# thanosDelatolas/eva-vos

Hardware: AMD Instinct MI355X
Metric: frames/sec STCN mask-propagate 480p 1-obj (higher is better)
Workload: dtype f32; 1 GPU; DAVIS-17-val-shaped 480x854 (padded 480x864) single-object STCN propagate: fresh engine, interact(mask,0), T=66 frames/video, mem_freq=5, top_k=50; one video per step per GPU; videos_per_gpu=38, streams_per_gpu=4, key_lookahead=0, clips=8 distinct synthetic clips (one per pooled engine), weights=synthetic recipe seed 0 (no checkpoints offline)

## Files before the change

eva_vos_amd/csrc/engine.cpp:

```cpp
#include "engine.h"
#include "src_hash.h"

#include <algorithm>
#include <atomic>
#include <cmath>
#include <cstdarg>
#include <cstdio>
#include <cstdlib>
#include <cstring>
#include <map>
#include <mutex>
#include <unordered_map>
#include <utility>

namespace stcn {

static thread_local char g_err[512] = "";
void set_error(const char *fmt, ...) {
    va_list ap;
    va_start(ap, fmt);
    vsnprintf(g_err, sizeof(g_err), fmt, ap);
    va_end(ap);
}
const char *get_error() { return g_err; }

Knobs Knobs::from_env() {
    Knobs k;
    k.wino_min_cin = env_int("STCN_WINO_MIN_CIN", k.wino_min_cin);
    k.wino_ppw = env_int("STCN_WINO_PPW", k.wino_ppw);
    k.wino4_chunk_mb = env_int("STCN_WINO4_CHUNK_MB", k.wino4_chunk_mb);
    k.fusion_conv12 = env_int("STCN_FUSION_CONV12", k.fusion_conv12) != 0;
    k.fusion_wino = env_int("STCN_FUSION_WINO", k.fusion_wino) != 0;
    k.pw_chain = env_int("STCN_PW_CHAIN", k.pw_chain);
    return k;
}

void Prof::reset() {
    for (int i = 0; i < STCN_K_COUNT; ++i) { flops[i] = 0; bytes[i] = 0; exec_flops[i] = 0; launches[i] = 0; }
    hbm_conv_flops = hbm_conv_bytes = hbm_conv_ms = 0; hbm_conv_launches = 0;
    wino2_flops = wino4_flops = 0;
    for (auto &e : events) { pool.push_back(e.a); pool.push_back(e.b); }
    events.clear();
}
Prof::Ev &Prof::push_pair(int cls, bool hbm) {
    Ev e; e.cls = cls; e.hbm = hbm;
    for (hipEvent_t *p : {&e.a, &e.b}) {
        if (!pool.empty()) { *p = pool.back(); pool.pop_back(); }
        else (void)hipEventCreate(p);
// ... 357 lines not shown
    if ((rc = alloc((void **)&logit4, (size_t)kg * d.hw4 * sizeof(float)))) return rc;
    if ((rc = alloc((void **)&flogit, (size_t)k * d.npix * sizeof(float)))) return rc;
    if ((rc = alloc((void **)&agg, (size_t)(k + 1) * group * d.npix * sizeof(float)))) return rc;
    if ((rc = alloc((void **)&agg_alt, (size_t)(k + 1) * group * d.npix * sizeof(float)))) return rc;
    if ((rc = alloc((void **)&pooled, (size_t)std::max(20, attention_nchp(2 * (k + 1))) * d.hw16 * sizeof(float)))) return rc;
    if ((rc = alloc((void **)&amap, (size_t)(k + 1) * 2 * d.hw16 * sizeof(float)))) return rc;
    if ((rc = alloc((void **)&attn, (size_t)(k + 1) * 2 * d.npix * sizeof(float)))) return rc;
    const MemReadScratchSizes ms = memread_scratch_floats(group * d.hw16);
    if ((rc = alloc((void **)&cand_v, std::max(ms.cand_v, attention_part_floats(k + 1, d.hw16)) * sizeof(float)))) return rc;
    if ((rc = alloc((void **)&cand_i, ms.cand_i * sizeof(int32_t)))) return rc;
    if ((rc = alloc((void **)&cand_n, ms.cand_n * sizeof(int32_t)))) return rc;
    if ((rc = alloc((void **)&qk, (size_t)group * d.hw16 * 64 * sizeof(float)))) return rc;
    if ((rc = alloc((void **)&vin, (size_t)k * d.npix * 8 * sizeof(float)))) return rc;
    if ((rc = alloc((void **)&gmax, ms.gmax * sizeof(float)))) return rc;
    if ((rc = alloc((void **)&tau, ms.tau * sizeof(float)))) return rc;
    return STCN_OK;
}
void Work::release() {
    for (void *p : allocs) pool_free(p);
    allocs.clear();
}

static thread_local int g_fail_countdown = 0;
static thread_local int g_fail_reserve = 0;
static std::atomic<int> g_side_delay_us{0};
void inject_failure_after(int n) { g_fail_countdown = n; }
int launch_status(const char *what) {
    if (g_fail_countdown > 0 && --g_fail_countdown == 0) {
        (void)hipGetLastError();
        set_error("launch of '%s' failed: injected fault (stcn_test_fail_at)", what);
// ... 54 lines not shown
    p.x0_bytes = (unsigned)x0b;
    p.x1_bytes = (unsigned)x1b;
    p.w_bytes = (unsigned)((long)cw.cout * cw.Kp * 4);
    if (a.x1 && ((cw.cin_p % 32) || (c0 % 32) || cw.kh * cw.kw > 32)) { set_error("conv '%s': two-source input needs 32-aligned channel splits", name.c_str()); return STCN_E_INVALID; }
    p.w = cw.w; p.wino_u = cw.wino_u; p.wino4_u = cw.wino4_u;
    p.bias = cw.bias; p.res = a.res; p.res_bs = res_bs; p.res_bmod = a.res_bmod; p.y = a.y; p.y_bs = a.y_bs;
    p.relu_in = a.relu_in; p.relu_out = a.relu_out;
    p.fd_ohw = fastdiv_make((unsigned)(p.OH * p.OW));
    p.fd_ow = fastdiv_make((unsigned)p.OW);
    p.fd_cin = fastdiv_make((unsigned)p.Cin);
    p.fd_kw = fastdiv_make((unsigned)p.KW);
    p.pointwise = cw.kh == 1 && cw.kw == 1 && a.stride == 1 && !a.x1 && bs0 == (long)H * W * c0;
    p.affine_out = (a.y_bs == 0 || a.y_bs == (long)p.OH * p.OW * p.N) && (!a.res || (res_bs == (long)p.OH * p.OW * p.N && !a.res_bmod)) &&
                   ((long)p.M + 128) * p.N * 4 < (1L << 32);
    p.partial = w.splitk;
    p.kn = w.kn;
    pl = ConvPlan{};
    pl.fl = 2.0 * p.M * p.N * (double)(cw.kh * cw.kw * cw.cin);
    if (a.force_splitk <= 0 && (fusion_conv_plan(p, pl) || wino4_plan(p, m.wino4_min_wg, w.wino_v_floats, w.splitk_floats, pl) ||
                                wino_plan(p, w.wino_v_floats, w.splitk_floats, pl)))
        return STCN_OK;
    conv_plan(p, a.force_splitk, w.splitk_floats, pl);
    return STCN_OK;
}

int run_conv(const Model &m, Work &w, hipStream_t s, const std::string &name, const ConvArgs &a) {
    ConvP p;
    ConvPlan &pl = g_path.plan;
    const int rc = plan_conv(m, w, name, a, p, pl);
    if (rc) return rc;
// ... 485 lines not shown
    if (rc) { stcn_engine_destroy(e); return rc; }
    const Dims &d = e->d;
    for (int t = 0; t < T; ++t)
        pack_image_launch(images_dev + (size_t)t * 3 * H * W, e->images4 + (size_t)t * d.npix * 4, H, W, nh, nw, e->lw, e->lh, e->stream);
    if ((rc = engine_init_outputs(e))) { stcn_engine_destroy(e); return rc; }
    HIPCHK(hipStreamSynchronize(e->stream));
    *out = e;
    return STCN_OK;
}

int stcn_engine_reset(stcn_engine *e) {
    if (!e) { set_error("stcn_engine_reset: null engine"); return STCN_E_INVALID; }
    HIPCHK(hipSetDevice(e->model->device));
    if (e->side) HIPCHK(hipStreamSynchronize(e->side));
    if (e->stream2) HIPCHK(hipStreamSynchronize(e->stream2));
    e->failed.clear();
    e->interacted.clear();
    e->n_certain = 0;
    e->n_cached = 0;
    std::fill(e->slot_of.begin(), e->slot_of.end(), -1);
    std::fill(e->vparts_ready.begin(), e->vparts_ready.end(), 0);
    std::fill(e->key_pending.begin(), e->key_pending.end(), 0);
    e->fuse_pending[0] = e->fuse_pending[1] = 0;
    e->stats = stcn_stats{};
    return engine_init_outputs(e);
}

int stcn_engine_destroy(stcn_engine *e) {
    if (!e) return STCN_OK;
    if (e->stream) (void)hipStreamSynchronize(e->stream); else (void)hipDeviceSynchronize();
// ... 458 lines not shown
```

eva_vos_amd/csrc/engine.h:

```cpp
#pragma once
#include <hip/hip_runtime.h>

#include <deque>
#include <map>
#include <memory>
#include <set>
#include <string>
#include <vector>

#include "../../include/stcn_hip.h"
#include "kernels.h"

namespace stcn {

void set_error(const char *fmt, ...);
struct Model;
struct ConvW;
hipError_t pool_malloc(void **p, size_t bytes);
void pool_free(void *p);
void pool_release();
bool wants_wino(const ConvW &cw);
bool wants_wino4(const ConvW &cw);
bool wants_wino_fusion12(const ConvW &cw);
int make_wino(Model &m, ConvW &cw, const std::vector<float> &w_host);
// ... 69 lines not shown
    float *A = nullptr, *B = nullptr, *C = nullptr, *D = nullptr;
    float *splitk = nullptr; size_t splitk_floats = 0;
    float *wino_v = nullptr; size_t wino_v_floats = 0;
    float *cbam = nullptr;
    float *readout = nullptr;
    float *logit4 = nullptr;
    float *flogit = nullptr;
    float *agg = nullptr;
    float *agg_alt = nullptr;
    float *pooled = nullptr, *amap = nullptr, *attn = nullptr;
    float *cand_v = nullptr; int32_t *cand_i = nullptr, *cand_n = nullptr;
    float *gmax = nullptr, *tau = nullptr;
    int32_t *centre = nullptr;
    float *qk = nullptr;
    float *vin = nullptr;
    Prof *prof = nullptr;
    Knobs kn = Knobs::from_env();
    int conv_cls = STCN_K_CONV;
    std::vector<void *> allocs;
    int init(int nh, int nw, int k, int key_batch = 1, int group = 1);
    void release();
};

struct KeyOut { float *k16, *msq, *f16_thin, *f16, *s8, *s4, *f8_copy, *f4_copy, *dthin = nullptr, *cthin = nullptr; };
void inject_failure_after(int n);
int launch_status(const char *what);
const char *last_conv_path();
void set_conv_path(const char *s);
void conv_trace(int on);
const char *conv_trace_get();
constexpr long CONV_DENSE = -1;
struct ConvArgs {
    const float *x0 = nullptr, *x1 = nullptr;
    int c0 = 0, c1 = 0;
    long bs0 = CONV_DENSE, bs1 = 0;
    int B = 1, H = 0, W = 0, stride = 1;
// ... 86 lines not shown
```

eva_vos_amd/csrc/hooks.cpp:

```cpp
#include <algorithm>
#include <cmath>
#include <cstdlib>
#include <cstring>
#include <string>
#include <vector>

#include "engine.h"

using namespace stcn;
#define RC(x) do { int rc_ = (x); if (rc_) return rc_; } while (0)

namespace {
struct TmpWork {
    Work w;
    int rc;
    TmpWork(int nh, int nw, int k) { rc = w.init(nh, nw, k); }
    ~TmpWork() { (void)hipDeviceSynchronize(); w.release(); }
};
struct DevBuf {
    float *p = nullptr;
    int alloc(size_t floats) { HIPCHK(hipMalloc((void **)&p, floats * 4)); return STCN_OK; }
    ~DevBuf() { if (p) { (void)hipDeviceSynchronize(); (void)hipFree(p); } }
};
ConvW test_convw(int Cin, int Cout, int KH, int KW) {
    ConvW cw;
    cw.cout = Cout; cw.cin = Cin; cw.cin_p = Cin; cw.kh = KH; cw.kw = KW;
    cw.K = KH * KW * Cin; cw.Kp = (cw.K + 31) / 32 * 32;
    return cw;
}
size_t test_wino_v_floats(int B, int OH, int OW, int Cin) {
    const size_t v2 = (size_t)16 * Cin * (((size_t)B * ((OH + 1) / 2) * ((OW + 1) / 2) + 63) / 64 * 64);
    const size_t v4 = (size_t)36 * Cin * (((size_t)B * ((OH + 3) / 4) * ((OW + 3) / 4) + 127) / 128 * 128);
    return v2 > v4 ? v2 : v4;
}
struct ConvRig {
    Model m;
    Work w;
    DevBuf wv, ws;
    ~ConvRig() { (void)hipDeviceSynchronize(); for (void *p : m.allocs) (void)hipFree(p); }
    int init(ConvW cw, const std::vector<float> *hw, bool f4, int B, int OH, int OW, size_t slab_floats) {
        if (hw) {
            RC(make_wino(m, cw, *hw));
            RC(make_wino_fusion12(m, cw, *hw));
            if (f4) RC(make_wino4(m, cw, *hw));
            w.wino_v_floats = test_wino_v_floats(B, OH, OW, cw.cin_p);
            RC(wv.alloc(w.wino_v_floats));
            w.wino_v = wv.p;
        }
        m.conv["t"] = cw;
        w.splitk_floats = slab_floats;
        RC(ws.alloc(w.splitk_floats));
        w.splitk = ws.p;
        return STCN_OK;
    }
};
int plan_test_conv(int B, int H, int W, int Cin, int Cout, int K, int stride, int flags, int splitk, ConvP &p, ConvPlan &pl) {
    static float buf[4];
    Model m;
    ConvW cw = test_convw(Cin, Cout, K, K);
    cw.w = cw.bias = buf;
    const int OH = (H + 2 * (K / 2) - K) / stride + 1, OW = (W + 2 * (K / 2) - K) / stride + 1;
    Work w;
    if (K == 3 && stride == 1) {
        if (wants_wino(cw) || wants_wino_fusion12(cw)) cw.wino_u = buf;
        if (flags & 4) { if (wants_wino4(cw)) cw.wino4_u = buf; m.wino4_min_wg = 0; }
        w.wino_v_floats = test_wino_v_floats(B, OH, OW, Cin);
        w.wino_v = buf;
// ... 370 lines not shown
```

eva_vos_amd/csrc/kernels.h:

```cpp
#pragma once
#include <hip/hip_runtime.h>
#include <stdint.h>

#include <cstdlib>

#include "../../include/stcn_hip.h"

namespace stcn {

struct FastDiv {
    unsigned magic, shift, d;
};
static inline FastDiv fastdiv_make(unsigned d) {
    FastDiv f{0, 0, d};
    if (d <= 1) return f;
    unsigned s = 0;
    while ((1ull << s) < d) ++s;
    f.magic = (unsigned)(((1ull << (31 + s)) / d) + 1);
    f.shift = s - 1;
    return f;
}
#if defined(__HIPCC__)
__device__ __forceinline__ int fastdiv(int x, const FastDiv f) {
    return f.d <= 1 ? x : (int)(__umulhi((unsigned)x, f.magic) >> f.shift);
// ... 3 lines not shown
    return (xcd < r8 ? xcd * (q8 + 1) : r8 * (q8 + 1) + (xcd - r8) * q8) + (bid >> 3);
}
#endif

static inline int env_int(const char *name, int dflt) { const char *e = getenv(name); return e ? atoi(e) : dflt; }
static inline bool env_on(const char *name, bool dflt = true) { return env_int(name, dflt) != 0; }
int device_cus();

struct Knobs {
    int wino_min_cin = 128;
    int wino_ppw = 0;
    int wino4_chunk_mb = 160;
    int fusion_conv12 = 0;
    int fusion_wino = 1;
    int pw_chain = 2;
    static Knobs from_env();
};

struct ConvP {
    const float *x0, *x1;
    int c0, c1;
    long bs0, bs1;
    unsigned x0_bytes, x1_bytes, w_bytes;
    int B, H, W;
    int OH, OW;
    int KH, KW, stride, pad;
    int Cin;
    int M, N;
    int K, Kp;
    const float *w;
    const float *bias;
    const float *res;
    long res_bs;
    int res_bmod;
    float *y;
    long y_bs;
    int relu_in, relu_out;
    int splitk;
    float *partial;
    int rem_full, rem_split, rem_per;
    const float *wino_u;
    const float *wino4_u;
    FastDiv fd_ohw, fd_ow;
    FastDiv fd_cin, fd_kw;
    int pointwise;
    int affine_out;
    int tile_big;
    int panel;
    int chain;
    Knobs kn;
};
constexpr int W4_MAX_CHUNKS = 16;
struct WinoGeom { int TH, TW, Mt, Mt_pad, KB; };
struct W2Plan { int tiles_n, ntile, kb_per_split; };
struct W4Plan { int tiles_m, tiles_n, mb, grid, full_wg, pieces, per, chunks, tm_per_chunk, judge_wg; };
enum ConvFamily { CONV_LITERAL = 0, CONV_FUSION = 1, CONV_WINO4 = 2, CONV_WINO2 = 3, CONV_DIRECT = 4 };
struct ConvPlan {
    int family = CONV_LITERAL;
    bool fusion_wino = false;
    WinoGeom geo{};
    W4Plan w4{};
    W2Plan w2{};
    int splitk = 1;
    int ppw = 0;
    const char *variant = "";
    bool tail = false;
// ... 109 lines not shown
```

eva_vos_amd/csrc/winograd4.hip:

```cpp
#include <hip/hip_ext.h>

#include <cstdio>
#include <cstdlib>
#include <type_traits>

#include "wino_common.h"

namespace stcn {

typedef float f32x4 __attribute__((ext_vector_type(4)));
typedef float f32x16 __attribute__((ext_vector_type(16)));

#ifdef STCN_W4_CLOCK
__device__ unsigned long long g_w4_clock[2 * 8192];
#if STCN_W4_CLOCK == 2
#define W4_MFMA(a_, b_, c_) w4_fake_mfma(a_, b_, c_)
#endif
#endif
#ifndef W4_MFMA
#define W4_MFMA(a_, b_, c_) __builtin_amdgcn_mfma_f32_32x32x2f32(a_, b_, c_, 0, 0, 0)
#endif

static constexpr int W4T = 32;
static constexpr int W4N = 32;
// ... 72 lines not shown
}

struct Wino4G {
    const float *V, *U;
    unsigned v_bytes, u_bytes;
    int Mt, Mt_pad, KB, N;
    int TH, TW, OH, OW, B, M;
    const float *bias, *res;
    long res_bs; int res_bmod;
    float *y; long y_bs;
    int relu_out;
    FastDiv fd_tpi, fd_tw, fd_tiles_n;
    int full_wg, pieces, kb_per_piece;
    float *partial;
    int tm0;
    int xb_m, xb_n, xb_cols;
};

template <int MB>
__global__ __launch_bounds__(64 * W4W) void wino4_gemm_kernel(const Wino4G p, const int tiles_n) {
    constexpr int PPW = 3, WT = W4T * MB;
    extern __shared__ __attribute__((aligned(16))) float smem[];
    int swz, piece = -1, kb0 = 0, kb1 = p.KB;
    if (MB == 1 && p.pieces > 1 && (int)blockIdx.x >= p.full_wg) {
        const int j = xcd_contiguous_block((int)blockIdx.x - p.full_wg, (int)gridDim.x - p.full_wg);
        const int rt = j / p.pieces;
        piece = j - rt * p.pieces;
        swz = p.full_wg + rt;
        kb0 = piece * p.kb_per_piece;
        kb1 = min(p.KB, kb0 + p.kb_per_piece);
    } else {
        swz = xcd_contiguous_block((int)blockIdx.x, MB == 1 && p.pieces > 1 ? p.full_wg : (int)gridDim.x);
    }
    int tm_l = fastdiv(swz, p.fd_tiles_n), tn = swz - tm_l * tiles_n;
    if (p.xb_m > 0 && piece < 0) {
        const int per = p.xb_m * p.xb_n, blk = swz / per, in = swz - blk * per;
        const int bm_i = blk / p.xb_cols, bn_i = blk - bm_i * p.xb_cols, im = in / p.xb_n;
        tm_l = bm_i * p.xb_m + im;
        tn = bn_i * p.xb_n + (in - im * p.xb_n);
    }
    const int tm = tm_l + p.tm0;
    const int t = threadIdx.x, lane = t & 63, l31 = lane & 31, h = lane >> 5;
    const int wave = __builtin_amdgcn_readfirstlane(t >> 6);
    const int pos0 = PPW * wave;

    const __amdgpu_buffer_rsrc_t rv = __builtin_amdgcn_make_buffer_rsrc(const_cast<float *>(p.V), 0, p.v_bytes, 0x00020000);
    const __amdgpu_buffer_rsrc_t ru = __builtin_amdgcn_make_buffer_rsrc(const_cast<float *>(p.U), 0, p.u_bytes, 0x00020000);
    const unsigned vl = (unsigned)(l31 * 32 + h * 16);
    unsigned sa0[PPW], sb0[PPW];
#pragma unroll
    for (int pi = 0; pi < PPW; ++pi) {
        sa0[pi] = (unsigned)((((long)(pos0 + pi) * p.KB + kb0) * p.Mt_pad + tm * WT) * 32);
        sb0[pi] = (unsigned)((((long)(pos0 + pi) * p.KB + kb0) * p.N + tn * W4N) * 32);
    }
    const unsigned sa = (unsigned)p.Mt_pad * 32u, sb = (unsigned)p.N * 32u;

    f32x16 acc[PPW][MB];
#pragma unroll
    for (int pi = 0; pi < PPW; ++pi)
#pragma unroll
        for (int bi = 0; bi < MB; ++bi)
#pragma unroll
            for (int e = 0; e < 16; ++e) acc[pi][bi][e] = 0.f;

    const int nk = kb1 - kb0;
    auto load1 = [&](int k, int pi, f32x4 (&fa)[MB], f32x4 &fb) {
        const unsigned oa = sa0[pi] + (unsigned)k * sa, ob = sb0[pi] + (unsigned)k * sb;
#pragma unroll
        for (int bi = 0; bi < MB; ++bi) fa[bi] = __builtin_bit_cast(f32x4, __builtin_amdgcn_raw_buffer_load_b128(rv, vl, oa + bi * 1024u, 0));
        fb = __builtin_bit_cast(f32x4, __builtin_amdgcn_raw_buffer_load_b128(ru, vl, ob, 0));
    };
    auto compute1 = [&](int pi, const f32x4 (&fa)[MB], const f32x4 &fb) {
#pragma unroll
        for (int j = 0; j < 4; ++j)
#pragma unroll
            for (int bi = 0; bi < MB; ++bi) acc[pi][bi] = W4_MFMA(fa[bi][j], fb[j], acc[pi][bi]);
    };
#ifdef STCN_W4_CLOCK
    unsigned long long ck_t0 = 0, ck_r0 = 0;
    if (wave == 0) {
        __builtin_amdgcn_sched_barrier(0);
        ck_t0 = __builtin_amdgcn_s_memtime();
        ck_r0 = __builtin_amdgcn_s_memrealtime();
        __builtin_amdgcn_s_waitcnt(0xC07F);
        __builtin_amdgcn_sched_barrier(0);
    }
#endif
    if (MB == 1) {
        f32x4 fa[3][PPW][MB], fb[3][PPW];
        auto load = [&](int k, int set) {
#pragma unroll
            for (int pi = 0; pi < PPW; ++pi) load1(k, pi, fa[set][pi], fb[set][pi]);
        };
        auto compute = [&](int set) {
#pragma unroll
            for (int j = 0; j < 4; ++j)
#pragma unroll
                for (int pi = 0; pi < PPW; ++pi)
#pragma unroll
                    for (int bi = 0; bi < MB; ++bi)
                        acc[pi][bi] = W4_MFMA(fa[set][pi][bi][j], fb[set][pi][j], acc[pi][bi]);
        };
        load(0, 0);
        load(min(1, nk - 1), 1);
        int k = 0;
        for (; k + 2 < nk; k += 3) {
            load(k + 2, 2);
            __builtin_amdgcn_sched_barrier(0);
            compute(0);
            __builtin_amdgcn_sched_barrier(0);
            load(min(k + 3, nk - 1), 0);
            __builtin_amdgcn_sched_barrier(0);
            compute(1);
            __builtin_amdgcn_sched_barrier(0);
            load(min(k + 4, nk - 1), 1);
            __builtin_amdgcn_sched_barrier(0);
            compute(2);
            __builtin_amdgcn_sched_barrier(0);
        }
        if (k < nk) compute(0);
        if (k + 1 < nk) compute(1);
    } else {
        f32x4 fa[2][PPW], fb[2][PPW];
        auto loadA = [&](int k, int bi, f32x4 (&d)[PPW]) {
#pragma unroll
            for (int pi = 0; pi < PPW; ++pi)
                d[pi] = __builtin_bit_cast(f32x4, __builtin_amdgcn_raw_buffer_load_b128(rv, vl, sa0[pi] + (unsigned)k * sa + bi * 1024u, 0));
        };
        auto loadB = [&](int k, f32x4 (&d)[PPW]) {
#pragma unroll
            for (int pi = 0; pi < PPW; ++pi)
                d[pi] = __builtin_bit_cast(f32x4, __builtin_amdgcn_raw_buffer_load_b128(ru, vl, sb0[pi] + (unsigned)k * sb, 0));
        };
        auto comp = [&](int bi, const f32x4 (&a)[PPW], const f32x4 (&bb)[PPW]) {
#pragma unroll
            for (int j = 0; j < 4; ++j)
#pragma unroll
                for (int pi = 0; pi < PPW; ++pi) acc[pi][bi] = W4_MFMA(a[pi][j], bb[pi][j], acc[pi][bi]);
        };
        loadB(0, fb[0]);
        loadA(0, 0, fa[0]);
        for (int k = 0; k < nk; k += 2) {
            const int k2 = min(k + 2, nk - 2);
            loadA(k, 1, fa[1]);
            __builtin_amdgcn_sched_barrier(0);
            comp(0, fa[0], fb[0]);
            __builtin_amdgcn_sched_barrier(0);
            loadB(k + 1, fb[1]);
            loadA(k + 1, 0, fa[0]);
            __builtin_amdgcn_sched_barrier(0);
            comp(1, fa[1], fb[0]);
            __builtin_amdgcn_sched_barrier(0);
            loadA(k + 1, 1, fa[1]);
            __builtin_amdgcn_sched_barrier(0);
            comp(0, fa[0], fb[1]);
            __builtin_amdgcn_sched_barrier(0);
            loadB(k2, fb[0]);
            loadA(k2, 0, fa[0]);
            __builtin_amdgcn_sched_barrier(0);
            comp(1, fa[1], fb[1]);
            __builtin_amdgcn_sched_barrier(0);
        }
    }
#ifdef STCN_W4_CLOCK
    if (wave == 0) {
        __builtin_amdgcn_sched_barrier(0);
        const unsigned long long ck_t1 = __builtin_amdgcn_s_memtime(), ck_r1 = __builtin_amdgcn_s_memrealtime();
        __builtin_amdgcn_s_waitcnt(0xC07F);
        __builtin_amdgcn_sched_barrier(0);
        if (lane == 0 && blockIdx.x < 8192) { g_w4_clock[2 * blockIdx.x] = ck_t1 - ck_t0; g_w4_clock[2 * blockIdx.x + 1] = ck_r1 - ck_r0; }
    }
#endif
    const int chq = t & 7, tl = (t >> 3) & 31;
    const int jh = __builtin_amdgcn_readfirstlane(t >> 8);
    const int tpi = p.TH * p.TW, ohw = p.OH * p.OW;
    const int n = tn * W4N + 4 * chq;
    const bool kpiece = MB == 1 && piece >= 0;
    const float lo = p.relu_out ? 0.f : -__builtin_inff();
    const __amdgpu_buffer_rsrc_t rres = __builtin_amdgcn_make_buffer_rsrc(const_cast<float *>(p.res ? p.res : p.y), 0, -1, 0x00020000);
    const __amdgpu_buffer_rsrc_t ry = __builtin_amdgcn_make_buffer_rsrc(p.y, 0, -1, 0x00020000);
    const unsigned y_bs = (unsigned)(p.y_bs ? p.y_bs : (long)ohw * p.N);
#pragma unroll
    for (int half = 0; half < MB; ++half) {
        int toff = 32 * half + tl;
        asm volatile("" : "+v"(toff));
        const long gt = (long)tm * WT + toff;
        const bool work = jh < 2 && gt < p.Mt;
        const int gtc = (int)min(gt, (long)p.Mt - 1);
        const int b = fastdiv(gtc, p.fd_tpi);
        const int rr = gtc - b * tpi;
        const int ty = fastdiv(rr, p.fd_tw), tx = rr - ty * p.TW;
        unsigned prow[4], pcol[2];
#pragma unroll
        for (int i2 = 0; i2 < 4; ++i2) prow[i2] = (unsigned)(min(4 * ty + i2, p.OH - 1) * p.OW * p.N) * 4u;
#pragma unroll
        for (int j = 0; j < 2; ++j) pcol[j] = (unsigned)(min(4 * tx + 2 * jh + j, p.OW - 1) * p.N + n) * 4u;
        if (half) __syncthreads();
#pragma unroll
        for (int pi = 0; pi < PPW; ++pi)
#pragma unroll
            for (int r = 0; r < 16; ++r)
                smem[((pos0 + pi) * W4T + (r & 3) + 8 * (r >> 2) + 4 * h) * W4N + l31] = acc[pi][half][r];
        f32x4 yv[2][4], bv = {0.f, 0.f, 0.f, 0.f};
        if (p.bias && !kpiece) {
            int nb = n;
            asm volatile("" : "+v"(nb));
            bv = *reinterpret_cast<const f32x4 *>(p.bias + nb);
        }
        if (p.res && !kpiece && jh < 2) {
            const unsigned rb = (unsigned)(p.res_bmod ? b % p.res_bmod : b) * (unsigned)p.res_bs * 4u;
#pragma unroll
            for (int j = 0; j < 2; ++j)
#pragma unroll
                for (int i2 = 0; i2 < 4; ++i2)
                    yv[j][i2] = __builtin_bit_cast(f32x4, __builtin_amdgcn_raw_buffer_load_b128(rres, rb + prow[i2] + pcol[j], 0, 0));
        } else {
#pragma unroll
            for (int j = 0; j < 2; ++j)
#pragma unroll
                for (int i2 = 0; i2 < 4; ++i2) yv[j][i2] = f32x4{0.f, 0.f, 0.f, 0.f};
        }
        __syncthreads();
        if (!work) continue;
        auto zrow = [&](int xi, auto JH, f32x4 (&zr)[2]) {
            f32x4 m[6];
            int ro4 = (xi * 6 * W4T + tl) * (W4N / 4) + chq;
            asm volatile("" : "+v"(ro4));
#pragma unroll
            for (int nu = 0; nu < 6; ++nu) m[nu] = reinterpret_cast<const f32x4 *>(smem)[ro4 + nu * W4T * (W4N / 4)];
            if (decltype(JH)::value == 0) {
                zr[0] = m[0] + (m[1] + m[2]) + (m[3] + m[4]);
                zr[1] = (m[1] - m[2]) * 0.75f + (m[3] - m[4]) * 1.5f;
            } else {
                zr[0] = (m[1] + m[2]) * 0.5625f + (m[3] + m[4]) * 2.25f;
                zr[1] = (m[1] - m[2]) * 0.421875f + (m[3] - m[4]) * 3.375f + m[5];
            }
        };
        auto columns = [&](auto JH) {
            f32x4 za[2];
#pragma unroll
            for (int j = 0; j < 2; ++j)
#pragma unroll
// ... 19 lines not shown
            zrow(5, JH, za);
#pragma unroll
            for (int j = 0; j < 2; ++j) yv[j][3] += za[j];
        };
        if (jh == 0) columns(std::integral_constant<int, 0>{});
        else columns(std::integral_constant<int, 1>{});
        if (kpiece) {
            float *dst = p.partial + (((long)(swz - p.full_wg) * p.pieces + piece) * W4T + tl) * (16 * W4N) + 4 * chq;
#pragma unroll
            for (int j = 0; j < 2; ++j)
#pragma unroll
                for (int i2 = 0; i2 < 4; ++i2) *reinterpret_cast<f32x4 *>(dst + (i2 * 4 + 2 * jh + j) * W4N) = yv[j][i2];
            continue;
        }
        const unsigned yb = (unsigned)b * y_bs * 4u;
#pragma unroll
        for (int j = 0; j < 2; ++j)
#pragma unroll
            for (int i2 = 0; i2 < 4; ++i2) {
#pragma unroll
                for (int c = 0; c < 4; ++c) yv[j][i2][c] = fmaxf(yv[j][i2][c], lo);
                const bool ok = 4 * tx + 2 * jh + j < p.OW && 4 * ty + i2 < p.OH;
                __builtin_amdgcn_raw_buffer_store_b128(__builtin_bit_cast(__attribute__((__vector_size__(4 * sizeof(unsigned)))) unsigned, yv[j][i2]), ry,
                                                       ok ? yb + prow[i2] + pcol[j] : 0xFFFFFFFFu, 0, 0);
            }
    }
}

__global__ __launch_bounds__(256) void wino4_reduce_kernel(const Wino4G p, const int tiles_n) {
    const int rt = blockIdx.x >> 6, swz = p.full_wg + rt;
    const int tm = fastdiv(swz, p.fd_tiles_n), tn = swz - tm * tiles_n;
    const int n_l = threadIdx.x & 31;
    const int e = ((blockIdx.x & 63) << 3) + (threadIdx.x >> 5);
    const int tl = e >> 4, px = e & 15;
    const int n = tn * W4N + n_l;
    const long gt = (long)tm * W4T + tl;
    if (gt >= p.Mt) return;
    const int tpi = p.TH * p.TW, ohw = p.OH * p.OW;
    const int b = fastdiv((int)gt, p.fd_tpi);
    const int rr = (int)(gt - (long)b * tpi);
// ... 95 lines not shown
    g.xb_m = g.xb_n = g.xb_cols = 0;
    {
        const int rows = pl.full_wg / tiles_n;
        if (pl.chunks == 1 && pl.full_wg % 8 == 0 && rows * tiles_n == pl.full_wg && tiles_n >= 8) {
            const int per = pl.full_wg / 8;
            int best = 0, best_sum = per % tiles_n == 0 ? per / tiles_n + tiles_n : rows + tiles_n;
            for (int bn = 2; bn <= tiles_n; ++bn) {
                if (per % bn || tiles_n % bn) continue;
                const int bm = per / bn;
                if (bm < 1 || rows % bm || (rows / bm) * (tiles_n / bn) != 8) continue;
                if (bm + bn < best_sum) { best_sum = bm + bn; best = bn; }
            }
            if (best && best != tiles_n) { g.xb_n = best; g.xb_m = per / best; g.xb_cols = tiles_n / best; }
        }
    }
    const size_t lds = (size_t)36 * W4T * W4N * sizeof(float);
    for (int c = 0; c < pl.chunks; ++c) {
        const int tm_lo = c * pl.tm_per_chunk, tm_hi = tm_lo + pl.tm_per_chunk < tiles_m ? tm_lo + pl.tm_per_chunk : tiles_m;
        const int tile_lo = tm_lo * W4T * mb, tile_hi = pl.chunks == 1 ? ge.Mt_pad : tm_hi * W4T * mb;
        hipEvent_t *ei = ev_in ? ev_in[c] : nullptr, *eg = ev_gemm ? ev_gemm[c] : nullptr;
        const WinoInGrid ig = wino_input_grid(tile_hi - tile_lo, p.Cin);
        launch(wino4_input_kernel, dim3(ig.gx, ig.chunks), dim3(256), 0, s, ei, p.x0, p.x0_bytes, p.bs0, p.H, p.W, p.Cin, p.relu_in, ge.TH, ge.TW,
               ge.Mt, ge.Mt_pad, ig.per, tile_lo, tile_hi, V);
        g.tm0 = tm_lo;
        if (mb == 2) {
            const int grid = (tm_hi - tm_lo) * tiles_n;
            launch(wino4_gemm_kernel<2>, dim3(grid), dim3(64 * W4W), lds, s, eg, g, tiles_n);
        } else {
            launch(wino4_gemm_kernel<1>, dim3(pl.grid), dim3(64 * W4W), lds, s, eg, g, tiles_n);
            if (g.pieces > 1) launch(wino4_reduce_kernel, dim3((tiles_m * tiles_n - g.full_wg) * 64), dim3(256), 0, s, ev_red, g, tiles_n);
        }
    }
}

void wino4_transform_weights(const float *w, int N, int Cin, int Kp, float *U) {
    static const double G[6][3] = {{64.0 / 81, 0, 0},
                                   {-128.0 / 243, -32.0 / 81, -8.0 / 27},
                                   {-128.0 / 243, 32.0 / 81, -8.0 / 27},
                                   {32.0 / 243, 16.0 / 81, 8.0 / 27},
                                   {32.0 / 243, -16.0 / 81, 8.0 / 27},
                                   {0, 0, 1}};
    wino_transform_weights_with(G, w, N, Cin, Kp, U);
}

// ... 8 lines not shown
```

Baseline: 820.1 frames/s.

## Make Winograd-4 GEMM persistent with per-XCD atomic work queue and prefetch

Launches the F(4x4,3x3) Winograd GEMM with at most one workgroup per CU and lets each workgroup pull further tiles from a per-XCD atomic counter. The next tile's first operand loads are issued during the current tile's epilogue so they overlap the output transform. This is meant to remove launch/tail overhead of many small workgroups and hide the fill latency of each tile. In exchange it adds atomics, a ticket in LDS, extra barriers, register pressure from the wider state, and a queue that must be reset between runs.

```diff
diff --git a/eva_vos_amd/csrc/engine.cpp b/eva_vos_amd/csrc/engine.cpp
--- a/eva_vos_amd/csrc/engine.cpp
+++ b/eva_vos_amd/csrc/engine.cpp
@@ -32,6 +32,7 @@
     k.fusion_conv12 = env_int("STCN_FUSION_CONV12", k.fusion_conv12) != 0;
     k.fusion_wino = env_int("STCN_FUSION_WINO", k.fusion_wino) != 0;
     k.pw_chain = env_int("STCN_PW_CHAIN", k.pw_chain);
+    k.wino4_walk = env_int("STCN_WINO4_WALK", k.wino4_walk);
     return k;
 }
 
@@ -419,6 +420,13 @@
     if ((rc = alloc((void **)&vin, (size_t)k * d.npix * 8 * sizeof(float)))) return rc;
     if ((rc = alloc((void **)&gmax, ms.gmax * sizeof(float)))) return rc;
     if ((rc = alloc((void **)&tau, ms.tau * sizeof(float)))) return rc;
+    if ((rc = alloc((void **)&wino4_queue, W4_QUEUE_WORDS * sizeof(int)))) return rc;
+    HIPCHK(hipMemsetAsync(wino4_queue, 0, W4_QUEUE_WORDS * sizeof(int), nullptr));
+    HIPCHK(hipStreamSynchronize(nullptr));
+    return STCN_OK;
+}
+int Work::reset_queue(hipStream_t s) {
+    if (wino4_queue) HIPCHK(hipMemsetAsync(wino4_queue, 0, W4_QUEUE_WORDS * sizeof(int), s));
     return STCN_OK;
 }
 void Work::release() {
@@ -503,6 +511,7 @@
     p.affine_out = (a.y_bs == 0 || a.y_bs == (long)p.OH * p.OW * p.N) && (!a.res || (res_bs == (long)p.OH * p.OW * p.N && !a.res_bmod)) &&
                    ((long)p.M + 128) * p.N * 4 < (1L << 32);
     p.partial = w.splitk;
+    p.wino4_queue = w.wino4_queue;
     p.kn = w.kn;
     pl = ConvPlan{};
     pl.fl = 2.0 * p.M * p.N * (double)(cw.kh * cw.kw * cw.cin);
@@ -1018,6 +1027,9 @@
     HIPCHK(hipSetDevice(e->model->device));
     if (e->side) HIPCHK(hipStreamSynchronize(e->side));
     if (e->stream2) HIPCHK(hipStreamSynchronize(e->stream2));
+    if (int rc = e->work.reset_queue(e->stream)) return rc;
+    if (int rc = e->work_side.reset_queue(e->side)) return rc;
+    if (int rc = e->work2.reset_queue(e->stream2)) return rc;
     e->failed.clear();
     e->interacted.clear();
     e->n_certain = 0;
diff --git a/eva_vos_amd/csrc/engine.h b/eva_vos_amd/csrc/engine.h
--- a/eva_vos_amd/csrc/engine.h
+++ b/eva_vos_amd/csrc/engine.h
@@ -107,12 +107,14 @@
     int32_t *centre = nullptr;
     float *qk = nullptr;
     float *vin = nullptr;
+    int *wino4_queue = nullptr;
     Prof *prof = nullptr;
     Knobs kn = Knobs::from_env();
     int conv_cls = STCN_K_CONV;
     std::vector<void *> allocs;
     int init(int nh, int nw, int k, int key_batch = 1, int group = 1);
     void release();
+    int reset_queue(hipStream_t s);
 };
 
 struct KeyOut { float *k16, *msq, *f16_thin, *f16, *s8, *s4, *f8_copy, *f4_copy, *dthin = nullptr, *cthin = nullptr; };
diff --git a/eva_vos_amd/csrc/hooks.cpp b/eva_vos_amd/csrc/hooks.cpp
--- a/eva_vos_amd/csrc/hooks.cpp
+++ b/eva_vos_amd/csrc/hooks.cpp
@@ -36,7 +36,7 @@
 struct ConvRig {
     Model m;
     Work w;
-    DevBuf wv, ws;
+    DevBuf wv, ws, wq;
     ~ConvRig() { (void)hipDeviceSynchronize(); for (void *p : m.allocs) (void)hipFree(p); }
     int init(ConvW cw, const std::vector<float> *hw, bool f4, int B, int OH, int OW, size_t slab_floats) {
         if (hw) {
@@ -51,6 +51,10 @@
         w.splitk_floats = slab_floats;
         RC(ws.alloc(w.splitk_floats));
         w.splitk = ws.p;
+        RC(wq.alloc(W4_QUEUE_WORDS));
+        HIPCHK(hipMemset(wq.p, 0, W4_QUEUE_WORDS * sizeof(int)));
+        HIPCHK(hipDeviceSynchronize());
+        w.wino4_queue = reinterpret_cast<int *>(wq.p);
         return STCN_OK;
     }
 };
diff --git a/eva_vos_amd/csrc/kernels.h b/eva_vos_amd/csrc/kernels.h
--- a/eva_vos_amd/csrc/kernels.h
+++ b/eva_vos_amd/csrc/kernels.h
@@ -41,6 +41,7 @@
     int fusion_conv12 = 0;
     int fusion_wino = 1;
     int pw_chain = 2;
+    int wino4_walk = 1;
     static Knobs from_env();
 };
 
@@ -65,6 +66,7 @@
     int relu_in, relu_out;
     int splitk;
     float *partial;
+    int *wino4_queue;
     int rem_full, rem_split, rem_per;
     const float *wino_u;
     const float *wino4_u;
@@ -77,6 +79,7 @@
     int chain;
     Knobs kn;
 };
+constexpr int W4_QUEUE_WORDS = 9;
 constexpr int W4_MAX_CHUNKS = 16;
 struct WinoGeom { int TH, TW, Mt, Mt_pad, KB; };
 struct W2Plan { int tiles_n, ntile, kb_per_split; };
diff --git a/eva_vos_amd/csrc/winograd4.hip b/eva_vos_amd/csrc/winograd4.hip
--- a/eva_vos_amd/csrc/winograd4.hip
+++ b/eva_vos_amd/csrc/winograd4.hip
@@ -110,48 +110,124 @@
     int full_wg, pieces, kb_per_piece;
     float *partial;
     int tm0;
+    int n_items;
+    int *queue;
     int xb_m, xb_n, xb_cols;
+    FastDiv fd_pieces, fd_xb_per, fd_xb_cols, fd_xb_n, fd_res_bmod;
+};
+
+struct W4Item {
+    int swz, piece, kb0, kb1, tm, tn;
+    unsigned sa0[3], sb0[3];
 };
 
 template <int MB>
 __global__ __launch_bounds__(64 * W4W) void wino4_gemm_kernel(const Wino4G p, const int tiles_n) {
     constexpr int PPW = 3, WT = W4T * MB;
+    constexpr int TICKET = 36 * W4T * W4N;
+    constexpr int LEAD = MB == 1 ? 6 : 4;
     extern __shared__ __attribute__((aligned(16))) float smem[];
-    int swz, piece = -1, kb0 = 0, kb1 = p.KB;
-    if (MB == 1 && p.pieces > 1 && (int)blockIdx.x >= p.full_wg) {
-        const int j = xcd_contiguous_block((int)blockIdx.x - p.full_wg, (int)gridDim.x - p.full_wg);
-        const int rt = j / p.pieces;
-        piece = j - rt * p.pieces;
-        swz = p.full_wg + rt;
-        kb0 = piece * p.kb_per_piece;
-        kb1 = min(p.KB, kb0 + p.kb_per_piece);
-    } else {
-        swz = xcd_contiguous_block((int)blockIdx.x, MB == 1 && p.pieces > 1 ? p.full_wg : (int)gridDim.x);
-    }
-    int tm_l = fastdiv(swz, p.fd_tiles_n), tn = swz - tm_l * tiles_n;
-    if (p.xb_m > 0 && piece < 0) {
-        const int per = p.xb_m * p.xb_n, blk = swz / per, in = swz - blk * per;
-        const int bm_i = blk / p.xb_cols, bn_i = blk - bm_i * p.xb_cols, im = in / p.xb_n;
-        tm_l = bm_i * p.xb_m + im;
-        tn = bn_i * p.xb_n + (in - im * p.xb_n);
-    }
-    const int tm = tm_l + p.tm0;
-    const int t = threadIdx.x, lane = t & 63, l31 = lane & 31, h = lane >> 5;
-    const int wave = __builtin_amdgcn_readfirstlane(t >> 6);
+    const int wave = __builtin_amdgcn_readfirstlane((int)threadIdx.x >> 6);
+    auto tid = [&]() {
+        unsigned z = 0;
+        asm volatile("" : "+v"(z));
+        return wave * 64 + (int)__builtin_amdgcn_mbcnt_hi(~0u, __builtin_amdgcn_mbcnt_lo(~0u, z));
+    };
     const int pos0 = PPW * wave;
+    const int G = (int)gridDim.x, xq = (int)blockIdx.x & 7;
+    const bool walk = p.n_items > G;
+
+    auto decode = [&](int vb) {
+        W4Item it;
+        it.piece = -1; it.kb0 = 0; it.kb1 = p.KB;
+        if (MB == 1 && p.pieces > 1 && vb >= p.full_wg) {
+            const int j = xcd_contiguous_block(vb - p.full_wg, p.n_items - p.full_wg);
+            const int rt = fastdiv(j, p.fd_pieces);
+            it.piece = j - rt * p.pieces;
+            it.swz = p.full_wg + rt;
+            it.kb0 = it.piece * p.kb_per_piece;
+            it.kb1 = min(p.KB, it.kb0 + p.kb_per_piece);
+        } else {
+            it.swz = xcd_contiguous_block(vb, MB == 1 && p.pieces > 1 ? p.full_wg : p.n_items);
+        }
+        int tm_l = fastdiv(it.swz, p.fd_tiles_n);
+        it.tn = it.swz - tm_l * tiles_n;
+        if (p.xb_m > 0 && it.piece < 0) {
+            const int per = p.xb_m * p.xb_n, blk = fastdiv(it.swz, p.fd_xb_per), in = it.swz - blk * per;
+            const int bm_i = fastdiv(blk, p.fd_xb_cols), bn_i = blk - bm_i * p.xb_cols, im = fastdiv(in, p.fd_xb_n);
+            tm_l = bm_i * p.xb_m + im;
+            it.tn = bn_i * p.xb_n + (in - im * p.xb_n);
+        }
+        it.tm = tm_l + p.tm0;
+#pragma unroll
+        for (int pi = 0; pi < PPW; ++pi) {
+            it.sa0[pi] = (unsigned)((((long)(pos0 + pi) * p.KB + it.kb0) * p.Mt_pad + it.tm * WT) * 32);
+            it.sb0[pi] = (unsigned)((((long)(pos0 + pi) * p.KB + it.kb0) * p.N + it.tn * W4N) * 32);
+        }
+        return it;
+    };
+    auto pull = [&]() {
+        unsigned z = 0;
+        asm volatile("" : "+v"(z));
+        return __hip_atomic_fetch_add(p.queue + xq + z, 1, __ATOMIC_RELAXED, __HIP_MEMORY_SCOPE_AGENT);
+    };
 
     const __amdgpu_buffer_rsrc_t rv = __builtin_amdgcn_make_buffer_rsrc(const_cast<float *>(p.V), 0, p.v_bytes, 0x00020000);
     const __amdgpu_buffer_rsrc_t ru = __builtin_amdgcn_make_buffer_rsrc(const_cast<float *>(p.U), 0, p.u_bytes, 0x00020000);
-    const unsigned vl = (unsigned)(l31 * 32 + h * 16);
-    unsigned sa0[PPW], sb0[PPW];
-#pragma unroll
-    for (int pi = 0; pi < PPW; ++pi) {
-        sa0[pi] = (unsigned)((((long)(pos0 + pi) * p.KB + kb0) * p.Mt_pad + tm * WT) * 32);
-        sb0[pi] = (unsigned)((((long)(pos0 + pi) * p.KB + kb0) * p.N + tn * W4N) * 32);
-    }
+    unsigned vl = 0;
     const unsigned sa = (unsigned)p.Mt_pad * 32u, sb = (unsigned)p.N * 32u;
 
+    constexpr int NSET = MB == 1 ? 3 : 2;
+    f32x4 fa[NSET][PPW], fb[NSET][PPW];
     f32x16 acc[PPW][MB];
+    auto load = [&](const W4Item &it, int k, int set) {
+#pragma unroll
+        for (int pi = 0; pi < PPW; ++pi) {
+            fa[set][pi] = __builtin_bit_cast(f32x4, __builtin_amdgcn_raw_buffer_load_b128(rv, vl, it.sa0[pi] + (unsigned)k * sa, 0));
+            fb[set][pi] = __builtin_bit_cast(f32x4, __builtin_amdgcn_raw_buffer_load_b128(ru, vl, it.sb0[pi] + (unsigned)k * sb, 0));
+        }
+    };
+    auto compute = [&](int set) {
+#pragma unroll
+        for (int j = 0; j < 4; ++j)
+#pragma unroll
+            for (int pi = 0; pi < PPW; ++pi) acc[pi][0] = W4_MFMA(fa[set][pi][j], fb[set][pi][j], acc[pi][0]);
+    };
+    auto loadA = [&](const W4Item &it, int k, int bi, f32x4 (&d)[PPW]) {
+#pragma unroll
+        for (int pi = 0; pi < PPW; ++pi)
+            d[pi] = __builtin_bit_cast(f32x4, __builtin_amdgcn_raw_buffer_load_b128(rv, vl, it.sa0[pi] + (unsigned)k * sa + bi * 1024u, 0));
+    };
+    auto loadB = [&](const W4Item &it, int k, f32x4 (&d)[PPW]) {
+#pragma unroll
+        for (int pi = 0; pi < PPW; ++pi)
+            d[pi] = __builtin_bit_cast(f32x4, __builtin_amdgcn_raw_buffer_load_b128(ru, vl, it.sb0[pi] + (unsigned)k * sb, 0));
+    };
+    auto comp = [&](int bi, const f32x4 (&a)[PPW], const f32x4 (&bb)[PPW]) {
+#pragma unroll
+        for (int j = 0; j < 4; ++j)
+#pragma unroll
+            for (int pi = 0; pi < PPW; ++pi) acc[pi][bi] = W4_MFMA(a[pi][j], bb[pi][j], acc[pi][bi]);
+    };
+    auto first_loads = [&](const W4Item &it) {
+        const int tl2 = tid();
+        vl = (unsigned)((tl2 & 31) * 32 + ((tl2 >> 5) & 1) * 16);
+        if constexpr (MB == 1) {
+            load(it, 0, 0);
+            __builtin_amdgcn_sched_barrier(0);
+            load(it, min(1, it.kb1 - it.kb0 - 1), 1);
+            __builtin_amdgcn_sched_barrier(0);
+        } else {
+            loadB(it, 0, fb[0]);
+            loadA(it, 0, 0, fa[0]);
+        }
+    };
+
+    W4Item cur = decode((int)blockIdx.x), nx = cur;
+    first_loads(cur);
+    int nvb = p.n_items;
+    for (bool again = false;; again = true) {
+    const int swz = cur.swz, piece = cur.piece, tm = cur.tm, tn = cur.tn;
 #pragma unroll
     for (int pi = 0; pi < PPW; ++pi)
 #pragma unroll
@@ -159,19 +235,11 @@
 #pragma unroll
             for (int e = 0; e < 16; ++e) acc[pi][bi][e] = 0.f;
 
-    const int nk = kb1 - kb0;
-    auto load1 = [&](int k, int pi, f32x4 (&fa)[MB], f32x4 &fb) {
-        const unsigned oa = sa0[pi] + (unsigned)k * sa, ob = sb0[pi] + (unsigned)k * sb;
-#pragma unroll
-        for (int bi = 0; bi < MB; ++bi) fa[bi] = __builtin_bit_cast(f32x4, __builtin_amdgcn_raw_buffer_load_b128(rv, vl, oa + bi * 1024u, 0));
-        fb = __builtin_bit_cast(f32x4, __builtin_amdgcn_raw_buffer_load_b128(ru, vl, ob, 0));
-    };
-    auto compute1 = [&](int pi, const f32x4 (&fa)[MB], const f32x4 &fb) {
-#pragma unroll
-        for (int j = 0; j < 4; ++j)
-#pragma unroll
-            for (int bi = 0; bi < MB; ++bi) acc[pi][bi] = W4_MFMA(fa[bi][j], fb[j], acc[pi][bi]);
-    };
+    const int nk = cur.kb1 - cur.kb0;
+    constexpr int STEP = MB == 1 ? 3 : 2;
+    const int kpull = !walk ? -2 : (nk - STEP - LEAD >= STEP ? (nk - STEP - LEAD) / STEP * STEP : -1);
+    int pulled = 0;
+    if (kpull == -1 && wave == 0 && tid() == 0) pulled = pull();
 #ifdef STCN_W4_CLOCK
     unsigned long long ck_t0 = 0, ck_r0 = 0;
     if (wave == 0) {
@@ -182,34 +250,19 @@
         __builtin_amdgcn_sched_barrier(0);
     }
 #endif
-    if (MB == 1) {
-        f32x4 fa[3][PPW][MB], fb[3][PPW];
-        auto load = [&](int k, int set) {
-#pragma unroll
-            for (int pi = 0; pi < PPW; ++pi) load1(k, pi, fa[set][pi], fb[set][pi]);
-        };
-        auto compute = [&](int set) {
-#pragma unroll
-            for (int j = 0; j < 4; ++j)
-#pragma unroll
-                for (int pi = 0; pi < PPW; ++pi)
-#pragma unroll
-                    for (int bi = 0; bi < MB; ++bi)
-                        acc[pi][bi] = W4_MFMA(fa[set][pi][bi][j], fb[set][pi][j], acc[pi][bi]);
-        };
-        load(0, 0);
-        load(min(1, nk - 1), 1);
+    if constexpr (MB == 1) {
         int k = 0;
         for (; k + 2 < nk; k += 3) {
-            load(k + 2, 2);
+            if (k == kpull && wave == 0) { if (tid() == 0) pulled = pull(); }
+            load(cur, k + 2, 2);
             __builtin_amdgcn_sched_barrier(0);
             compute(0);
             __builtin_amdgcn_sched_barrier(0);
-            load(min(k + 3, nk - 1), 0);
+            load(cur, min(k + 3, nk - 1), 0);
             __builtin_amdgcn_sched_barrier(0);
             compute(1);
             __builtin_amdgcn_sched_barrier(0);
-            load(min(k + 4, nk - 1), 1);
+            load(cur, min(k + 4, nk - 1), 1);
             __builtin_amdgcn_sched_barrier(0);
             compute(2);
             __builtin_amdgcn_sched_barrier(0);
@@ -217,42 +270,24 @@
         if (k < nk) compute(0);
         if (k + 1 < nk) compute(1);
     } else {
-        f32x4 fa[2][PPW], fb[2][PPW];
-        auto loadA = [&](int k, int bi, f32x4 (&d)[PPW]) {
-#pragma unroll
-            for (int pi = 0; pi < PPW; ++pi)
-                d[pi] = __builtin_bit_cast(f32x4, __builtin_amdgcn_raw_buffer_load_b128(rv, vl, sa0[pi] + (unsigned)k * sa + bi * 1024u, 0));
-        };
-        auto loadB = [&](int k, f32x4 (&d)[PPW]) {
-#pragma unroll
-            for (int pi = 0; pi < PPW; ++pi)
-                d[pi] = __builtin_bit_cast(f32x4, __builtin_amdgcn_raw_buffer_load_b128(ru, vl, sb0[pi] + (unsigned)k * sb, 0));
-        };
-        auto comp = [&](int bi, const f32x4 (&a)[PPW], const f32x4 (&bb)[PPW]) {
-#pragma unroll
-            for (int j = 0; j < 4; ++j)
-#pragma unroll
-                for (int pi = 0; pi < PPW; ++pi) acc[pi][bi] = W4_MFMA(a[pi][j], bb[pi][j], acc[pi][bi]);
-        };
-        loadB(0, fb[0]);
-        loadA(0, 0, fa[0]);
         for (int k = 0; k < nk; k += 2) {
             const int k2 = min(k + 2, nk - 2);
-            loadA(k, 1, fa[1]);
+            if (k == kpull && wave == 0) { if (tid() == 0) pulled = pull(); }
+            loadA(cur, k, 1, fa[1]);
             __builtin_amdgcn_sched_barrier(0);
             comp(0, fa[0], fb[0]);
             __builtin_amdgcn_sched_barrier(0);
-            loadB(k + 1, fb[1]);
-            loadA(k + 1, 0, fa[0]);
+            loadB(cur, k + 1, fb[1]);
+            loadA(cur, k + 1, 0, fa[0]);
             __builtin_amdgcn_sched_barrier(0);
             comp(1, fa[1], fb[0]);
             __builtin_amdgcn_sched_barrier(0);
-            loadA(k + 1, 1, fa[1]);
+            loadA(cur, k + 1, 1, fa[1]);
             __builtin_amdgcn_sched_barrier(0);
             comp(0, fa[0], fb[1]);
             __builtin_amdgcn_sched_barrier(0);
-            loadB(k2, fb[0]);
-            loadA(k2, 0, fa[0]);
+            loadB(cur, k2, fb[0]);
+            loadA(cur, k2, 0, fa[0]);
             __builtin_amdgcn_sched_barrier(0);
             comp(1, fa[1], fb[1]);
             __builtin_amdgcn_sched_barrier(0);
@@ -264,15 +299,15 @@
         const unsigned long long ck_t1 = __builtin_amdgcn_s_memtime(), ck_r1 = __builtin_amdgcn_s_memrealtime();
         __builtin_amdgcn_s_waitcnt(0xC07F);
         __builtin_amdgcn_sched_barrier(0);
-        if (lane == 0 && blockIdx.x < 8192) { g_w4_clock[2 * blockIdx.x] = ck_t1 - ck_t0; g_w4_clock[2 * blockIdx.x + 1] = ck_r1 - ck_r0; }
+        if ((threadIdx.x & 63) == 0 && blockIdx.x < 8192) { g_w4_clock[2 * blockIdx.x] = ck_t1 - ck_t0; g_w4_clock[2 * blockIdx.x + 1] = ck_r1 - ck_r0; }
     }
 #endif
-    const int chq = t & 7, tl = (t >> 3) & 31;
-    const int jh = __builtin_amdgcn_readfirstlane(t >> 8);
+    const int te = tid();
+    const int chq = te & 7, tl = (te >> 3) & 31, el31 = te & 31, eh = (te >> 5) & 1;
+    const int jh = __builtin_amdgcn_readfirstlane(te >> 8);
     const int tpi = p.TH * p.TW, ohw = p.OH * p.OW;
     const int n = tn * W4N + 4 * chq;
     const bool kpiece = MB == 1 && piece >= 0;
-    const float lo = p.relu_out ? 0.f : -__builtin_inff();
     const __amdgpu_buffer_rsrc_t rres = __builtin_amdgcn_make_buffer_rsrc(const_cast<float *>(p.res ? p.res : p.y), 0, -1, 0x00020000);
     const __amdgpu_buffer_rsrc_t ry = __builtin_amdgcn_make_buffer_rsrc(p.y, 0, -1, 0x00020000);
     const unsigned y_bs = (unsigned)(p.y_bs ? p.y_bs : (long)ohw * p.N);
@@ -287,16 +322,20 @@
         const int rr = gtc - b * tpi;
         const int ty = fastdiv(rr, p.fd_tw), tx = rr - ty * p.TW;
         unsigned prow[4], pcol[2];
-#pragma unroll
-        for (int i2 = 0; i2 < 4; ++i2) prow[i2] = (unsigned)(min(4 * ty + i2, p.OH - 1) * p.OW * p.N) * 4u;
-#pragma unroll
-        for (int j = 0; j < 2; ++j) pcol[j] = (unsigned)(min(4 * tx + 2 * jh + j, p.OW - 1) * p.N + n) * 4u;
-        if (half) __syncthreads();
+        auto offsets = [&](int ty_, int tx_) {
+#pragma unroll
+            for (int i2 = 0; i2 < 4; ++i2) prow[i2] = (unsigned)(min(4 * ty_ + i2, p.OH - 1) * p.OW * p.N) * 4u;
+#pragma unroll
+            for (int j = 0; j < 2; ++j) pcol[j] = (unsigned)(min(4 * tx_ + 2 * jh + j, p.OW - 1) * p.N + n) * 4u;
+        };
+        offsets(ty, tx);
+        if (half || again) __syncthreads();
 #pragma unroll
         for (int pi = 0; pi < PPW; ++pi)
 #pragma unroll
             for (int r = 0; r < 16; ++r)
-                smem[((pos0 + pi) * W4T + (r & 3) + 8 * (r >> 2) + 4 * h) * W4N + l31] = acc[pi][half][r];
+                smem[((pos0 + pi) * W4T + (r & 3) + 8 * (r >> 2) + 4 * eh) * W4N + el31] = acc[pi][half][r];
+        if (half == 0 && walk && wave == 0 && (te & 63) == 0) reinterpret_cast<int *>(smem)[TICKET] = pulled;
         f32x4 yv[2][4], bv = {0.f, 0.f, 0.f, 0.f};
         if (p.bias && !kpiece) {
             int nb = n;
@@ -304,7 +343,7 @@
             bv = *reinterpret_cast<const f32x4 *>(p.bias + nb);
         }
         if (p.res && !kpiece && jh < 2) {
-            const unsigned rb = (unsigned)(p.res_bmod ? b % p.res_bmod : b) * (unsigned)p.res_bs * 4u;
+            const unsigned rb = (unsigned)(p.res_bmod ? b - fastdiv(b, p.fd_res_bmod) * p.res_bmod : b) * (unsigned)p.res_bs * 4u;
 #pragma unroll
             for (int j = 0; j < 2; ++j)
 #pragma unroll
@@ -317,11 +356,27 @@
                 for (int i2 = 0; i2 < 4; ++i2) yv[j][i2] = f32x4{0.f, 0.f, 0.f, 0.f};
         }
         __syncthreads();
+        if (half == MB - 1) {
+            nvb = walk ? G + 8 * __builtin_amdgcn_readfirstlane(reinterpret_cast<const int *>(smem)[TICKET]) + xq : p.n_items;
+            if (nvb < p.n_items) {
+                nx = decode(nvb);
+                __builtin_amdgcn_sched_barrier(0);
+                first_loads(nx);
+            } else {
+#pragma unroll
+                for (int pi = 0; pi < PPW; ++pi) {
+                    fa[0][pi] = fb[0][pi] = f32x4{0.f, 0.f, 0.f, 0.f};
+                    if (MB == 1) fa[1][pi] = fb[1][pi] = f32x4{0.f, 0.f, 0.f, 0.f};
+                }
+            }
+            __builtin_amdgcn_sched_barrier(0);
+        }
         if (!work) continue;
         auto zrow = [&](int xi, auto JH, f32x4 (&zr)[2]) {
             f32x4 m[6];
-            int ro4 = (xi * 6 * W4T + tl) * (W4N / 4) + chq;
+            int ro4 = tl * (W4N / 4) + chq;
             asm volatile("" : "+v"(ro4));
+            ro4 += xi * 6 * W4T * (W4N / 4);
 #pragma unroll
             for (int nu = 0; nu < 6; ++nu) m[nu] = reinterpret_cast<const f32x4 *>(smem)[ro4 + nu * W4T * (W4N / 4)];
             if (decltype(JH)::value == 0) {
@@ -371,16 +426,30 @@
             continue;
         }
         const unsigned yb = (unsigned)b * y_bs * 4u;
+        int ty2 = ty, tx2 = tx;
+        asm volatile("" : "+v"(ty2), "+v"(tx2));
+        offsets(ty2, tx2);
+        int relu = p.relu_out;
+        asm volatile("" : "+s"(relu));
+        const float lo = relu ? 0.f : -__builtin_inff();
 #pragma unroll
         for (int j = 0; j < 2; ++j)
 #pragma unroll
             for (int i2 = 0; i2 < 4; ++i2) {
 #pragma unroll
                 for (int c = 0; c < 4; ++c) yv[j][i2][c] = fmaxf(yv[j][i2][c], lo);
-                const bool ok = 4 * tx + 2 * jh + j < p.OW && 4 * ty + i2 < p.OH;
+                const bool ok = 4 * tx2 + 2 * jh + j < p.OW && 4 * ty2 + i2 < p.OH;
                 __builtin_amdgcn_raw_buffer_store_b128(__builtin_bit_cast(__attribute__((__vector_size__(4 * sizeof(unsigned)))) unsigned, yv[j][i2]), ry,
                                                        ok ? yb + prow[i2] + pcol[j] : 0xFFFFFFFFu, 0, 0);
             }
+    }
+    if (nvb >= p.n_items) break;
+    cur = nx;
+    }
+    if (walk && wave == 0 && tid() == 0) {
+        const int left = __hip_atomic_fetch_add(p.queue + 8, 1, __ATOMIC_RELAXED, __HIP_MEMORY_SCOPE_AGENT);
+        if (left == G - 1)
+            for (int i = 0; i < 9; ++i) __hip_atomic_store(p.queue + i, 0, __ATOMIC_RELAXED, __HIP_MEMORY_SCOPE_AGENT);
     }
 }
 
@@ -506,7 +575,15 @@
             if (best && best != tiles_n) { g.xb_n = best; g.xb_m = per / best; g.xb_cols = tiles_n / best; }
         }
     }
-    const size_t lds = (size_t)36 * W4T * W4N * sizeof(float);
+    g.fd_pieces = fastdiv_make((unsigned)g.pieces); g.fd_xb_per = fastdiv_make((unsigned)(g.xb_m * g.xb_n));
+    g.fd_xb_cols = fastdiv_make((unsigned)g.xb_cols); g.fd_xb_n = fastdiv_make((unsigned)g.xb_n);
+    g.fd_res_bmod = fastdiv_make((unsigned)(g.res_bmod > 0 ? g.res_bmod : 1));
+    const size_t lds = (size_t)36 * W4T * W4N * sizeof(float) + 16;
+    auto resident = [&](int n_items) {
+        const int walk = p.kn.wino4_walk, cap = walk >= 8 ? walk : device_cus();
+        return walk == 0 || !p.wino4_queue || cap < 8 || n_items <= cap ? n_items : cap / 8 * 8;
+    };
+    g.queue = p.wino4_queue;
     for (int c = 0; c < pl.chunks; ++c) {
         const int tm_lo = c * pl.tm_per_chunk, tm_hi = tm_lo + pl.tm_per_chunk < tiles_m ? tm_lo + pl.tm_per_chunk : tiles_m;
         const int tile_lo = tm_lo * W4T * mb, tile_hi = pl.chunks == 1 ? ge.Mt_pad : tm_hi * W4T * mb;
@@ -516,10 +593,11 @@
                ge.Mt, ge.Mt_pad, ig.per, tile_lo, tile_hi, V);
         g.tm0 = tm_lo;
         if (mb == 2) {
-            const int grid = (tm_hi - tm_lo) * tiles_n;
-            launch(wino4_gemm_kernel<2>, dim3(grid), dim3(64 * W4W), lds, s, eg, g, tiles_n);
+            g.n_items = (tm_hi - tm_lo) * tiles_n;
+            launch(wino4_gemm_kernel<2>, dim3(resident(g.n_items)), dim3(64 * W4W), lds, s, eg, g, tiles_n);
         } else {
-            launch(wino4_gemm_kernel<1>, dim3(pl.grid), dim3(64 * W4W), lds, s, eg, g, tiles_n);
+            g.n_items = pl.grid;
+            launch(wino4_gemm_kernel<1>, dim3(resident(g.n_items)), dim3(64 * W4W), lds, s, eg, g, tiles_n);
             if (g.pieces > 1) launch(wino4_reduce_kernel, dim3((tiles_m * tiles_n - g.full_wg) * 64), dim3(256), 0, s, ev_red, g, tiles_n);
         }
     }
```

New measurement: 825.5 frames/s, median of 3. About the same (+0.7%).
